# yuliangguo/OmniFusion

Measured on AMD Instinct MI355X. Metric: panoramas/sec at 512x1024 ERP, N=18 256^2 patches; equi2pers+pers2equi GB/s vs HBM peak, higher is better.
Workload: dtype f16x3 (fp16 hi/lo pairs, fp32 accumulate: fp32-class); 1 GPU; cfg2/cfg4 shard: 8 panoramas/GPU/step, 512x1024 ERP, fov 80, nrows 4 (18 patches); full single-pass spherical_fusion forward (confidence=True) at patch size 128 — the only size the reference network exists at (SURVEY 0.1); random-init weights (seed 42); inputs resident in HBM; resample pair at 18x256^2 reported in roofline_resample; per_gpu_batch=8, global_batch=8, parallelism=image-sharded x1, execution=3 forwards in flight per GPU on 3 streams (spherical_fusion.pipelined)

## Files before the change

### omnifusion_amd/csrc/omni_conv_sh.hip

```cpp
#include "omni_conv_sh_common.h"

namespace {

__constant__ float wino_coef[16][4] = {
    {1, 0, 0, 0}, {1, 1, 0, 0}, {1, -1, 0, 0}, {0, -1, 0, 0},
    {1, 0, 1, 0}, {1, 1, 1, 1}, {1, -1, 1, -1}, {0, -1, 0, -1},
    {1, 0, -1, 0}, {1, 1, -1, -1}, {1, -1, -1, 1}, {0, -1, 0, 1},
    {0, 0, -1, 0}, {0, 0, -1, -1}, {0, 0, -1, 1}, {0, 0, 0, 1}};
template <int BM, int BN, int WM, int WN, int NST = 3, int NL = 0, bool PP = false, bool WINO = false, bool X1 = false>
__global__ __launch_bounds__(64 * (WM * WN + NL)) void conv_sh_kernel(ShConvArgs a)
{
    static_assert(!(WINO && X1), "Winograd: f16x3 only");
    static_assert(!PP || (NL > 0 && WM * WN == 8 && NST >= 3), "ping-pong: eight matrix waves (two per SIMD) + loader waves, three stages");
    static_assert(!WINO || (PP && BM / WM == 32 && BN / WN == 32), "Winograd: the ping-pong kernel with 32 x 32 wave tiles");
    constexpr int NW = WM * WN, LW = NL > 0 ? NL : NW, RPP = 8 * LW;
    constexpr int TM = BM / WM / 32, TN = BN / WN / 32;
    constexpr int APASS = BM / RPP, BPASS = BN / RPP, LPS = APASS + BPASS;
    static_assert(APASS >= 1 && BPASS >= 1, "a tile side must cover at least one DMA pass");
    constexpr int A_BYTES = BM * 128, STAGE = (BM + BN) * 128;
    __shared__ __attribute__((aligned(1024))) unsigned char lds[NST * STAGE];
    __shared__ long long cst[OMNI_ABL(32768) ? 256 : 1];
    const bool stamped = OMNI_ABL(32768) && blockIdx.x == 0 && blockIdx.y == 0 && a.ws != nullptr && a.splitk <= 1;
    auto cstamp = [&](int k) { if (OMNI_ABL(32768) && stamped && (threadIdx.x & 63) == 0 && k < 256) cst[k] = clock64(); };
    auto cdump = [&]() { if (OMNI_ABL(32768) && stamped && threadIdx.x == 0) for (int i = 0; i < 256; ++i) reinterpret_cast<long long*>(a.ws)[i] = cst[i]; };
// ... 453 lines not shown
#pragma unroll
    for (int d = 32; d > 0; d >>= 1) q += __shfl_xor(q, d);
    const float rstd = 1.0f / sqrtf(q * (1.0f / 512.0f) + eps);
    const f4v g0 = *reinterpret_cast<const f4v*>(g + lane * 4), g1 = *reinterpret_cast<const f4v*>(g + 256 + lane * 4);
    const f4v b0 = *reinterpret_cast<const f4v*>(b + lane * 4), b1 = *reinterpret_cast<const f4v*>(b + 256 + lane * 4);
    act_store4<SH>(y, o + lane * 4, v0 * rstd * g0 + b0);
    act_store4<SH>(y, o + 256 + lane * 4, v1 * rstd * g1 + b1);
}

__global__ __launch_bounds__(256) void sh_from_f32_kernel(const float* __restrict__ src, void* __restrict__ dst, size_t n4)
{
    const size_t i = (size_t)blockIdx.x * 256 + threadIdx.x;
    if (i >= n4) return;
    h4v hi, lo; sh_split4(*reinterpret_cast<const f4v*>(src + i * 4), hi, lo);
    unsigned char* dp = (unsigned char*)dst + sh_off(i * 4);
    *reinterpret_cast<h4v*>(dp) = hi; *reinterpret_cast<h4v*>(dp + 64) = lo;
}
__global__ __launch_bounds__(256) void sh_to_f32_kernel(const void* __restrict__ src, float* __restrict__ dst, size_t n4)
{
    const size_t i = (size_t)blockIdx.x * 256 + threadIdx.x;
    if (i >= n4) return;
    const unsigned char* sp = (const unsigned char*)src + sh_off(i * 4);
    *reinterpret_cast<f4v*>(dst + i * 4) = sh_join4(*reinterpret_cast<const h4v*>(sp), *reinterpret_cast<const h4v*>(sp + 64));
}

template <bool X1, int BM, int BN, int WM, int WN, int NST = 3, int NL = 0>
void launch_sh(ShConvArgs a, hipStream_t s)
{
    const int tiles = ((a.rows + BM - 1) / BM) * (a.Cout / BN);
    if constexpr (NL > 0 && WM * WN == 8) {
        if (omni_options().conv_pingpong) {
            hipLaunchKernelGGL((conv_sh_kernel<BM, BN, WM, WN, NST, NL, true, false, X1>), dim3(tiles, a.splitk > 1 ? a.splitk : 1), dim3(64 * (WM * WN + NL)), 0, s, a);
            return;
        }
    }
    hipLaunchKernelGGL((conv_sh_kernel<BM, BN, WM, WN, NST, NL, false, false, X1>), dim3(tiles, a.splitk > 1 ? a.splitk : 1), dim3(64 * (WM * WN + NL)), 0, s, a);
}

}

static int conv2d_sh_impl(const void* src1, const void* src2, const void* wt16, const float* bias,
                          const void* res, void* dst, int fmt, int M, int H, int W, int C1, int C2, int Cout,
                          int KH, int KW, int stride, int pad, int act, int splitk, float* ws, size_t ws_bytes,
                          const float* post, size_t post_elems, omni_stream_t stream, bool reduce = true);
extern "C" int omni_conv2d_sh_f16x3_ws(const void* src1, const void* src2, const void* wt16, const float* bias,
                                       const void* res, void* dst, int fmt, int M, int H, int W, int C1, int C2, int Cout,
                                       int KH, int KW, int stride, int pad, int act, int splitk, float* ws, size_t ws_bytes,
                                       omni_stream_t stream)
{
    return conv2d_sh_impl(src1, src2, wt16, bias, res, dst, fmt, M, H, W, C1, C2, Cout, KH, KW, stride, pad, act, splitk, ws, ws_bytes,
                          nullptr, 0, stream);
}
extern "C" int omni_conv2d_sh_f16x3_post_ws(const void* src1, const void* src2, const void* wt16, const float* bias,
                                            const void* res, void* dst, int fmt, int M, int H, int W, int C1, int C2, int Cout,
                                            int KH, int KW, int stride, int pad, int act, int splitk, float* ws, size_t ws_bytes,
                                            const float* post, size_t post_elems, omni_stream_t stream)
{
    return conv2d_sh_impl(src1, src2, wt16, bias, res, dst, fmt, M, H, W, C1, C2, Cout, KH, KW, stride, pad, act, splitk, ws, ws_bytes,
                          post, post_elems, stream);
}
extern "C" int omni_gemm_sh_f16x3_ln512_ws(const void* x, const void* wt16, const float* bias, const float* res, float* tok, const float* ln_g, const float* ln_b,
                                           float eps, void* y, int fmt, int rows, int K, int splitk, float* ws, size_t ws_bytes, omni_stream_t stream)
{
    if (!x || !wt16 || !tok || !ln_g || !ln_b || !y) OMNI_FAIL(OMNI_ERR_INVALID, "omni_gemm_sh_f16x3_ln512: null pointer");
    if (rows <= 0 || K <= 0 || K % 32) OMNI_FAIL(OMNI_ERR_INVALID, "omni_gemm_sh_f16x3_ln512: bad shape");
    if (fmt & 8) OMNI_FAIL(OMNI_ERR_UNSUPPORTED, "omni_gemm_sh_f16x3_ln512: no f16x1 form (fmt bit 3)");
    const int S = std::min(splitk, K / 32);
    if (S < 2) OMNI_FAIL(OMNI_ERR_INVALID, "omni_gemm_sh_f16x3_ln512: needs a split-K plan (splitk >= 2); an unsplit GEMM writes its result in its own epilogue");
    const int rc = conv2d_sh_impl(x, nullptr, wt16, bias, res, tok, 2, rows, 1, 1, K, 0, 512, 1, 1, 1, 0, OMNI_ACT_NONE, S, ws, ws_bytes, nullptr, 0, stream, false);
    if (rc != OMNI_OK) return rc;
    hipStream_t s = (hipStream_t)stream;
    if (fmt & 1) hipLaunchKernelGGL(sh_splitk_reduce_ln512_kernel<true>, dim3((rows + 3) / 4), dim3(256), 0, s, (const float*)ws, bias, res, tok, ln_g, ln_b, y, rows, S, (size_t)rows * 512, eps);
    else         hipLaunchKernelGGL(sh_splitk_reduce_ln512_kernel<false>, dim3((rows + 3) / 4), dim3(256), 0, s, (const float*)ws, bias, res, tok, ln_g, ln_b, y, rows, S, (size_t)rows * 512, eps);
    OMNI_HIP(hipGetLastError());
    return OMNI_OK;
}

template <bool X1>
static void conv_sh_select(const ShConvArgs& a, int fmt, hipStream_t s)
{
    const int KH = a.KH, KW = a.KW, stride = a.stride, pad = a.pad, H = a.H, W = a.W, M = a.M, Cout = a.Cout;
    const int ksteps = KH * KW * ((a.C1 + a.C2) / 32);
    const long long rows = a.rows;
    if (a.splitk <= 1 && KH == 3 && KW == 3 && stride == 1 && pad == 1 && H == W && (W == 16 || (W == 8 && omni_options().conv_img >= 2)) && rows % 128 == 0 &&
        Cout % 64 == 0 && !(fmt & 4) && omni_options().conv_img > 0 && !omni_options().conv_nohalo) {
        const int grid = (int)(rows / 128) * (Cout / 64);
        if (omni_options().conv_halo_bn == 32) {
            if (W == 16) omni_halo_launch(&a, 32, 4, false, 16, X1, 2 * grid, s);
            else         omni_halo_launch(&a, 32, 4, false, 8, X1, 2 * grid, s);
        }
        else if (W == 16) omni_halo_launch(&a, 64, 4, false, 16, X1, grid, s);
        else         omni_halo_launch(&a, 64, 4, false, 8, X1, grid, s);
        return;
    }
    if (a.splitk <= 1 && KH == 3 && KW == 3 && stride == 1 && pad == 1 && W % HT_W == 0 && H % 4 == 0 && !omni_options().conv_nohalo) {
        const int th = (H % 8 == 0 && omni_options().conv_halo_th == 8) ? 8 : 4;
        const int grid = M * (H / th) * (W / HT_W);
        if (th == 8) {
            if (Cout % 64 == 0 && omni_options().conv_halo_bn != 32) omni_halo_launch(&a, 64, 8, false, 0, X1, grid * (Cout / 64), s);
            else                omni_halo_launch(&a, 32, 8, false, 0, X1, grid * (Cout / 32), s);
        } else {
            const bool bn32 = omni_options().conv_halo_bn == 32 || ((fmt & 4) && omni_options().conv_halo_bn_lat == 32);
            if (Cout % 64 == 0 && !bn32) omni_halo_launch(&a, 64, 4, false, 0, X1, grid * (Cout / 64), s);
            else                omni_halo_launch(&a, 32, 4, false, 0, X1, grid * (Cout / 32), s);
        }
        return;
    }
    int tile = omni_options().conv_sh_tile;
    if (tile < 0) tile = 8;
    if (Cout % 64 != 0) launch_sh<X1, 128, 32, 4, 1>(a, s);
    else if (tile == 2 && Cout % 128 == 0) launch_sh<X1, 128, 128, 2, 2>(a, s);
    else if (tile == 1) launch_sh<X1, 128, 64, 2, 2>(a, s);
    else if (tile == 3) launch_sh<X1, 128, 64, 4, 2>(a, s);
    else if (tile == 4 && Cout % 128 == 0) launch_sh<X1, 128, 128, 4, 2>(a, s);
    else if (tile == 8 && Cout % 128 == 0 && ((rows + 255) / 256) * (long long)(Cout / 128) * a.splitk >= std::max(1, omni_options().conv_big_blocks)) launch_sh<X1, 256, 128, 4, 2>(a, s);
    else if (tile == 8 && Cout % 128 == 0 && ((rows + 127) / 128) * (long long)(Cout / 128) * a.splitk >= 128) launch_sh<X1, 128, 128, 4, 2, 3, 4>(a, s);
    else if (tile == 8 && ((rows + 127) / 128) * (long long)(Cout / 64) * a.splitk >= 128) launch_sh<X1, 128, 64, 4, 2, 3, 4>(a, s);
    else if (tile == 9 && Cout % 128 == 0 && ((rows + 255) / 256) * (long long)(Cout / 128) * a.splitk >= 128) launch_sh<X1, 256, 128, 4, 2>(a, s);
    else if (tile == 9 && Cout % 128 == 0 && ((rows + 127) / 128) * (long long)(Cout / 128) * a.splitk >= 128) launch_sh<X1, 128, 128, 4, 2>(a, s);
    else if (tile == 9 && ((rows + 127) / 128) * (long long)(Cout / 64) * a.splitk >= 128) launch_sh<X1, 128, 64, 4, 2>(a, s);
    else if (tile >= 5 && tile <= 7 && Cout % 128 == 0 && ((rows + 127) / 128) * (long long)(Cout / 128) * a.splitk >= (32ll << (tile - 4))) launch_sh<X1, 128, 128, 4, 2>(a, s);
    else if (tile >= 5 && tile <= 7 && ((rows + 127) / 128) * (long long)(Cout / 64) * a.splitk >= (32ll << (tile - 4))) launch_sh<X1, 128, 64, 4, 2>(a, s);
    else if (((rows + 63) / 64) * (long long)(Cout / 64) * a.splitk <= 256 && ksteps >= 8 && !omni_options().conv_nodeep) {
        if (omni_options().conv_deep_loaders) launch_sh<X1, 64, 64, 2, 2, 6, 4>(a, s);
        else launch_sh<X1, 64, 64, 2, 2, 6>(a, s);
    }
    else launch_sh<X1, 64, 64, 2, 2>(a, s);
}

static int conv2d_sh_impl(const void* src1, const void* src2, const void* wt16, const float* bias,
                          const void* res, void* dst, int fmt, int M, int H, int W, int C1, int C2, int Cout,
                          int KH, int KW, int stride, int pad, int act, int splitk, float* ws, size_t ws_bytes,
                          const float* post, size_t post_elems, omni_stream_t stream, bool reduce)
{
    const int dst_sh = fmt & 1;
    if (!src1 || !wt16 || !dst) OMNI_FAIL(OMNI_ERR_INVALID, "omni_conv2d_sh: null pointer");
    if (C1 <= 0 || C1 % 32 || C2 < 0 || C2 % 32 || Cout <= 0 || Cout % 32 || (C2 > 0 && !src2))
        OMNI_FAIL(OMNI_ERR_INVALID, "omni_conv2d_sh: channels must be multiples of 32");
    if (M <= 0 || H <= 0 || W <= 0 || KH <= 0 || KW <= 0 || KH > 3 || KW > 3 || stride <= 0 || pad < 0)
        OMNI_FAIL(OMNI_ERR_INVALID, "omni_conv2d_sh: bad shape (kernels up to 3x3)");
    ShConvArgs a;
    a.src1 = src1; a.src2 = src2; a.wt = wt16; a.bias = bias; a.res = res; a.dst = dst; a.dst_sh = dst_sh; a.res_f32 = (fmt >> 1) & 1;
    a.dbg = 0; a.noxcd = omni_options().conv_noxcd; a.wt_major = 0; a.epi_lds = omni_options().conv_epi_lds && !(fmt & 4);
#ifdef OMNI_DEBUG_BUILD
    a.dbg = omni_debug_bits("OMNI_CONV_DBG");
#endif
    a.M = M; a.H = H; a.W = W; a.C1 = C1; a.C2 = C2; a.Cout = Cout;
    a.KH = KH; a.KW = KW; a.stride = stride; a.pad = pad; a.act = act;
    a.Ho = (H + 2 * pad - KH) / stride + 1; a.Wo = (W + 2 * pad - KW) / stride + 1;
    const long long rows = (long long)M * a.Ho * a.Wo;
    if (rows <= 0 || rows >= (1ll << 31) || (long long)M * H * W >= (1ll << 31))
        OMNI_FAIL(OMNI_ERR_UNSUPPORTED, "omni_conv2d_sh: too many pixels for 32-bit row indices");
    a.rows = (int)rows;
    const int ksteps = KH * KW * ((C1 + C2) / 32);
    if ((long long)M * H * W * (C1 > C2 ? C1 : C2) * 4 >= (1ll << 31) || (long long)Cout * ksteps * 128 >= (1ll << 31))
        OMNI_FAIL(OMNI_ERR_UNSUPPORTED, "omni_conv2d_sh: an operand of 2 GiB or more (32-bit buffer offsets)");
    int S = splitk;
    if (S > ksteps) S = ksteps;
    if (S > 1 && (!ws || ws_bytes < (size_t)S * rows * Cout * sizeof(float)))
        OMNI_FAIL(OMNI_ERR_INVALID, "omni_conv2d_sh: split-K workspace too small");
    a.splitk = S > 1 ? S : 1; a.ws = ws;
    a.wt_major = omni_options().conv_wt_major == 2 || (omni_options().conv_wt_major == 1 &&
                 (long long)Cout * ksteps * 128 > (long long)M * H * W * (C1 + C2) * 4) ? 1 : 0;
    a.post = post; a.post_rows = 1; a.wino_th = a.wino_tw = a.wino_pix = 0;
    if (post) {
        if (Cout <= 0 || post_elems == 0 || post_elems % (size_t)Cout || post_elems / (size_t)Cout > 0x7fffffffull)
            OMNI_FAIL(OMNI_ERR_INVALID, "omni_conv2d_sh: the post-activation addend must hold whole rows of Cout channels");
        if (a.splitk > 1) OMNI_FAIL(OMNI_ERR_UNSUPPORTED, "omni_conv2d_sh: no post-activation addend with split-K");
        a.post_rows = (unsigned)(post_elems / (size_t)Cout);
    }
    hipStream_t s = (hipStream_t)stream;
    if (fmt & 8) conv_sh_select<true>(a, fmt, s);
    else         conv_sh_select<false>(a, fmt, s);
    OMNI_HIP(hipGetLastError());
    if (a.splitk > 1 && reduce) {
        const size_t n4 = (size_t)rows * Cout / 4;
        hipLaunchKernelGGL(sh_splitk_reduce_kernel, dim3((unsigned)((n4 + 255) / 256)), dim3(256), 0, s, (const float*)ws, bias, res, dst,
                           n4, Cout, a.splitk, (size_t)rows * Cout, act, a.dst_sh, a.res_f32);
        OMNI_HIP(hipGetLastError());
    }
    return OMNI_OK;
}

extern "C" int omni_splitk_reduce_ln512(const float* parts, int nparts, const float* bias, const float* res, float* tok, const float* lg, const float* lb,
                                        float eps, void* y, int fmt, int rows, omni_stream_t stream)
{
    if (!parts || nparts < 1 || !tok || !lg || !lb || !y || rows <= 0) OMNI_FAIL(OMNI_ERR_INVALID, "omni_splitk_reduce_ln512: null pointer or empty input");
    hipStream_t s = (hipStream_t)stream;
    if (fmt & 1) hipLaunchKernelGGL(sh_splitk_reduce_ln512_kernel<true>, dim3((rows + 3) / 4), dim3(256), 0, s, parts, bias, res, tok, lg, lb, y, rows, nparts, (size_t)rows * 512, eps);
    else         hipLaunchKernelGGL(sh_splitk_reduce_ln512_kernel<false>, dim3((rows + 3) / 4), dim3(256), 0, s, parts, bias, res, tok, lg, lb, y, rows, nparts, (size_t)rows * 512, eps);
    OMNI_HIP(hipGetLastError());
    return OMNI_OK;
}

OMNI_SH_OVERFLOW_ACCESSOR(omni_sh_overflow_conv)

extern "C" int omni_sh_overflow(int* flag, int reset)
{
    if (!flag) OMNI_FAIL(OMNI_ERR_INVALID, "omni_sh_overflow: null output");
    OMNI_HIP(hipDeviceSynchronize());
    unsigned v = 0;
    if (omni_sh_overflow_conv(&v, reset) != 0 || omni_sh_overflow_halo(&v, reset) != 0 || omni_sh_overflow_up2(&v, reset) != 0 ||
        omni_sh_overflow_rows(&v, reset) != 0 || omni_sh_overflow_net(&v, reset) != 0)
        OMNI_FAIL(OMNI_ERR_HIP, "omni_sh_overflow: could not read the device flag");
    *flag = v ? 1 : 0;
    return OMNI_OK;
}

extern "C" int omni_sh_from_f32(const float* src, void* dst, size_t n, omni_stream_t stream)
{
    if (!src || !dst || n % 32) OMNI_FAIL(OMNI_ERR_INVALID, "omni_sh_from_f32: null pointer or n % 32 != 0");
    if (n == 0) return OMNI_OK;
    hipLaunchKernelGGL(sh_from_f32_kernel, dim3((unsigned)((n / 4 + 255) / 256)), dim3(256), 0, (hipStream_t)stream, src, dst, n / 4);
    OMNI_HIP(hipGetLastError());
    return OMNI_OK;
}
extern "C" int omni_sh_to_f32(const void* src, float* dst, size_t n, omni_stream_t stream)
{
    if (!src || !dst || n % 32) OMNI_FAIL(OMNI_ERR_INVALID, "omni_sh_to_f32: null pointer or n % 32 != 0");
    if (n == 0) return OMNI_OK;
    hipLaunchKernelGGL(sh_to_f32_kernel, dim3((unsigned)((n / 4 + 255) / 256)), dim3(256), 0, (hipStream_t)stream, src, dst, n / 4);
    OMNI_HIP(hipGetLastError());
    return OMNI_OK;
}

namespace {

__global__ __launch_bounds__(256) void wino_input_sh_kernel(const void* __restrict__ src, void* __restrict__ V, int M, int H, int W, int C, size_t nt)
{
    const size_t i = (size_t)blockIdx.x * 256 + threadIdx.x;
    const int cq = C >> 2;
    if (i >= nt * cq) return;
    const size_t tl = i / cq;
    const int c = (int)(i - tl * cq) * 4;
    const int tw = W >> 1, th = H >> 1;
    const int m = (int)(tl / (size_t)(th * tw)), rem = (int)(tl - (size_t)m * th * tw), ty = rem / tw, tx = rem - ty * tw;
    f4v d[4][4];
#pragma unroll
    for (int a_ = 0; a_ < 4; ++a_)
#pragma unroll
        for (int b_ = 0; b_ < 4; ++b_) {
            const int y = 2 * ty - 1 + a_, x = 2 * tx - 1 + b_;
            d[a_][b_] = ((unsigned)y < (unsigned)H && (unsigned)x < (unsigned)W) ? act_load4<true>(src, (((size_t)m * H + y) * W + x) * C + c) : (f4v)(0.0f);
        }
    f4v u[4][4];
#pragma unroll
    for (int b_ = 0; b_ < 4; ++b_) { u[0][b_] = d[0][b_] - d[2][b_]; u[1][b_] = d[1][b_] + d[2][b_]; u[2][b_] = d[2][b_] - d[1][b_]; u[3][b_] = d[1][b_] - d[3][b_]; }
#pragma unroll
    for (int xi = 0; xi < 4; ++xi) {
        const f4v v0 = u[xi][0] - u[xi][2], v1 = u[xi][1] + u[xi][2], v2 = u[xi][2] - u[xi][1], v3 = u[xi][1] - u[xi][3];
        act_store4<true>(V, ((size_t)(4 * xi + 0) * nt + tl) * C + c, v0);
        act_store4<true>(V, ((size_t)(4 * xi + 1) * nt + tl) * C + c, v1);
        act_store4<true>(V, ((size_t)(4 * xi + 2) * nt + tl) * C + c, v2);
        act_store4<true>(V, ((size_t)(4 * xi + 3) * nt + tl) * C + c, v3);
    }
}

}

extern "C" int omni_wino_input_sh(const void* src, void* V, int M, int H, int W, int C, omni_stream_t stream)
{
    if (!src || !V) OMNI_FAIL(OMNI_ERR_INVALID, "omni_wino_input_sh: null pointer");
    if (M <= 0 || H <= 0 || W <= 0 || (H & 1) || (W & 1) || C <= 0 || C % 32) OMNI_FAIL(OMNI_ERR_INVALID, "omni_wino_input_sh: even image sides, channels a multiple of 32");
    const size_t nt = (size_t)M * (H / 2) * (W / 2), n = nt * (C / 4);
    if (16 * nt * C * 4 >= (1ull << 31)) OMNI_FAIL(OMNI_ERR_UNSUPPORTED, "omni_wino_input_sh: the transformed tensor must stay under 2 GiB (32-bit buffer offsets)");
    hipLaunchKernelGGL(wino_input_sh_kernel, dim3((unsigned)((n + 255) / 256)), dim3(256), 0, (hipStream_t)stream, src, V, M, H, W, C, nt);
    OMNI_HIP(hipGetLastError());
    return OMNI_OK;
}

extern "C" int omni_conv3x3_wino_sh_f16x3(const void* V, const void* wt16, const float* bias, const void* res, void* dst, int fmt,
                                          int M, int H, int W, int C, int Cout, int act, int splitk, float* ws, size_t ws_bytes, omni_stream_t stream)
{
    if (!V || !wt16 || !dst) OMNI_FAIL(OMNI_ERR_INVALID, "omni_conv3x3_wino_sh: null pointer");
    if (M <= 0 || H <= 0 || W <= 0 || (H & 1) || (W & 1) || C <= 0 || C % 32 || Cout <= 0 || Cout % 64) OMNI_FAIL(OMNI_ERR_INVALID, "omni_conv3x3_wino_sh: even image sides, C % 32 == 0, Cout % 64 == 0");
    if (splitk != 1 && splitk != 2 && splitk != 4) OMNI_FAIL(OMNI_ERR_INVALID, "omni_conv3x3_wino_sh: splitk must be 1, 2 or 4 (it divides the sixteen positions)");
    if (fmt & 8) OMNI_FAIL(OMNI_ERR_UNSUPPORTED, "omni_conv3x3_wino_sh: no f16x1 form (fmt bit 3)");
    const long long nt = (long long)M * (H / 2) * (W / 2), pix = (long long)M * H * W;
    if (16 * nt * C * 4 >= (1ll << 31) || (long long)Cout * 16 * C * 4 >= (1ll << 31) || pix >= (1ll << 31)) OMNI_FAIL(OMNI_ERR_UNSUPPORTED, "omni_conv3x3_wino_sh: an operand of 2 GiB or more");
    if (splitk > 1 && (!ws || ws_bytes < (size_t)splitk * pix * Cout * sizeof(float))) OMNI_FAIL(OMNI_ERR_INVALID, "omni_conv3x3_wino_sh: split workspace too small");
    ShConvArgs a;
    a.src1 = V; a.src2 = nullptr; a.wt = wt16; a.bias = bias; a.res = res; a.dst = dst; a.dst_sh = fmt & 1; a.res_f32 = (fmt >> 1) & 1;
    a.dbg = 0; a.noxcd = omni_options().conv_noxcd; a.wt_major = 0; a.epi_lds = 0;
    a.M = 1; a.H = 16; a.W = (int)nt; a.C1 = C; a.C2 = 0; a.Cout = Cout; a.KH = 16; a.KW = 1; a.stride = 1; a.pad = 0; a.act = act;
    a.Ho = H; a.Wo = W; a.rows = (int)nt; a.splitk = splitk; a.ws = ws; a.post = nullptr; a.post_rows = 1;
// ... 14 lines not shown
```

### omnifusion_amd/csrc/omni_conv_sh_common.h

```cpp
#pragma once
#include <stdlib.h>
#include <algorithm>
#include <type_traits>
#include "omni_internal.h"
#include "omni_sh.h"

#ifndef OMNI_CONV_ABL
#define OMNI_CONV_ABL 0
#endif
#define OMNI_ABL(bit) ((OMNI_CONV_ABL & (bit)) != 0)
#ifndef OMNI_PP_PRIO
#define OMNI_PP_PRIO 0
#endif
#ifndef OMNI_G1_PW
#define OMNI_G1_PW 4
#endif

namespace {

typedef float f16v __attribute__((ext_vector_type(16)));
typedef float f4v __attribute__((ext_vector_type(4)));
typedef _Float16 h8v __attribute__((ext_vector_type(8)));
typedef _Float16 h4v __attribute__((ext_vector_type(4)));
typedef _Float16 h2v __attribute__((ext_vector_type(2)));
// ... 117 lines not shown
                *reinterpret_cast<f4v*>(tile + px * PITCH + 32 * j + 8 * q + 4 * (lane >> 5)) = v;
            }
    }
    asm volatile("s_waitcnt lgkmcnt(0)" ::: "memory");
    constexpr int TASKS = 32 * NT * 4 / 64;
    constexpr int HALF = TASKS >= 4 ? TASKS / 2 : TASKS;
    const bool post = POST && a.post != nullptr;
#pragma unroll
    for (int k0 = 0; k0 < TASKS; k0 += HALF) {
        f4v va[HALF], vb[HALF], pa[HALF], pb[HALF]; h8v rh[HALF], rl[HALF];
        size_t off[HALF]; bool ok[HALF];
#pragma unroll
        for (int kk = 0; kk < HALF; ++kk) {
            const int task = (k0 + kk) * 64 + lane, px = task / (4 * NT), rem = task - px * (4 * NT), j = rem >> 2, pc = rem & 3;
            ok[kk] = px < nrows;
            va[kk] = *reinterpret_cast<const f4v*>(tile + px * PITCH + 32 * j + 8 * pc);
            vb[kk] = *reinterpret_cast<const f4v*>(tile + px * PITCH + 32 * j + 8 * pc + 4);
            off[kk] = ((px < 16 ? r0 + px : r1 + (px - 16)) * a.Cout + c0[j]) * 4 + 16 * pc;
            if (a.bias) { va[kk] += *reinterpret_cast<const f4v*>(a.bias + c0[j] + 8 * pc); vb[kk] += *reinterpret_cast<const f4v*>(a.bias + c0[j] + 8 * pc + 4); }
            if (a.res && ok[kk]) {
                rh[kk] = *reinterpret_cast<const h8v*>((const unsigned char*)a.res + off[kk]);
                rl[kk] = *reinterpret_cast<const h8v*>((const unsigned char*)a.res + off[kk] + 64);
            }
            if (post && ok[kk]) {
                const float* pp = a.post + (size_t)((unsigned)(px < 16 ? r0 + px : r1 + (px - 16)) % a.post_rows) * a.Cout + c0[j] + 8 * pc;
                pa[kk] = *reinterpret_cast<const f4v*>(pp); pb[kk] = *reinterpret_cast<const f4v*>(pp + 4);
            }
        }
#pragma unroll
        for (int kk = 0; kk < HALF; ++kk) {
            if (!ok[kk]) continue;
            f4v v0 = va[kk], v1 = vb[kk];
            if (a.res) {
#pragma unroll
                for (int e = 0; e < 4; ++e) { v0[e] += fmaf((float)rl[kk][e], 4.8828125e-4f, (float)rh[kk][e]); v1[e] += fmaf((float)rl[kk][4 + e], 4.8828125e-4f, (float)rh[kk][4 + e]); }
            }
            if (a.act == OMNI_ACT_RELU) {
#pragma unroll
                for (int e = 0; e < 4; ++e) { v0[e] = fmaxf(v0[e], 0.f); v1[e] = fmaxf(v1[e], 0.f); }
            } else if (a.act == OMNI_ACT_GELU) {
#pragma unroll
                for (int e = 0; e < 4; ++e) { v0[e] = 0.5f * v0[e] * (1.0f + erff(v0[e] * 0.70710678118654752440f)); v1[e] = 0.5f * v1[e] * (1.0f + erff(v1[e] * 0.70710678118654752440f)); }
            }
            if (post) { v0 += pa[kk]; v1 += pb[kk]; }
            h4v h0, l0, h1, l1;
            sh_split4(v0, h0, l0); sh_split4(v1, h1, l1);
            h8v oh, ol;
#pragma unroll
            for (int e = 0; e < 4; ++e) { oh[e] = h0[e]; oh[4 + e] = h1[e]; ol[e] = l0[e]; ol[4 + e] = l1[e]; }
            *reinterpret_cast<h8v*>((unsigned char*)a.dst + off[kk]) = oh;
            *reinterpret_cast<h8v*>((unsigned char*)a.dst + off[kk] + 64) = ol;
        }
    }
}

__device__ __forceinline__ void splitk_finish(f4v v, size_t o, const float* __restrict__ bias, const void* __restrict__ res, void* __restrict__ dst,
                                              int Cout, int act, int dst_sh, int res_f32)
{
    if (bias) v += *reinterpret_cast<const f4v*>(bias + (o % Cout));
    if (res && res_f32) v += *reinterpret_cast<const f4v*>((const float*)res + o);
    else if (res) {
        const unsigned char* rp = (const unsigned char*)res + sh_off(o);
        v += sh_join4(*reinterpret_cast<const h4v*>(rp), *reinterpret_cast<const h4v*>(rp + 64));
    }
    if (act == OMNI_ACT_RELU) { v.x = fmaxf(v.x, 0.f); v.y = fmaxf(v.y, 0.f); v.z = fmaxf(v.z, 0.f); v.w = fmaxf(v.w, 0.f); }
    else if (act == OMNI_ACT_GELU) {
#pragma unroll
        for (int e = 0; e < 4; ++e) v[e] = 0.5f * v[e] * (1.0f + erff(v[e] * 0.70710678118654752440f));
    }
    if (dst_sh) {
        h4v hi, lo; sh_split4(v, hi, lo);
        unsigned char* dp = (unsigned char*)dst + sh_off(o);
        *reinterpret_cast<h4v*>(dp) = hi; *reinterpret_cast<h4v*>(dp + 64) = lo;
    } else {
        *reinterpret_cast<f4v*>((float*)dst + o) = v;
    }
}

constexpr int HT_W = 32, HPW = HT_W + 2;

}

void omni_halo_launch(const void* args, int bn, int th, bool up2, int iw, bool x1, unsigned grid, hipStream_t s);
int omni_sh_overflow_halo(unsigned* out, int reset);
int omni_sh_overflow_up2(unsigned* out, int reset);
int omni_sh_overflow_rows(unsigned* out, int reset);
int omni_sh_overflow_net(unsigned* out, int reset);
```

### omnifusion_amd/csrc/omni_geometry.hip

```cpp
#include <math.h>
#include <stdlib.h>
#include <string.h>
#include <mutex>
#include <vector>
#include <memory>

#include "omni_internal.h"

static thread_local std::string g_err;
void omni_set_error(const std::string& msg) { g_err = msg; }
extern "C" const char* omni_last_error(void) { return g_err.c_str(); }
extern "C" int omni_version(void) { return OMNI_VERSION; }

namespace {
struct OptName { const char* name; const char* env; int OmniOptions::* field; int dflt; };
const OptName kOpts[] = {
    {"conv_sh_tile", "OMNI_CONV_SH_TILE", &OmniOptions::conv_sh_tile, -1},
    {"conv_nohalo", "OMNI_CONV_NOHALO", &OmniOptions::conv_nohalo, 0},
    {"conv_halo_th", "OMNI_CONV_HALO_TH", &OmniOptions::conv_halo_th, 4},
    {"conv_big_blocks", "OMNI_CONV_BIG_BLOCKS", &OmniOptions::conv_big_blocks, 128},
    {"conv_halo_bn_lat", "OMNI_CONV_HALO_BN_LAT", &OmniOptions::conv_halo_bn_lat, 32},
    {"conv_deep_loaders", "OMNI_CONV_DEEP_LOADERS", &OmniOptions::conv_deep_loaders, 1},
    {"conv_halo_up2_bn_lat", "OMNI_CONV_HALO_UP2_BN_LAT", &OmniOptions::conv_halo_up2_bn_lat, 64},
    {"conv_halo_bn", "OMNI_CONV_HALO_BN", &OmniOptions::conv_halo_bn, 64},
    {"conv_img", "OMNI_CONV_IMG", &OmniOptions::conv_img, 1},
    {"conv_nodeep", "OMNI_CONV_NODEEP", &OmniOptions::conv_nodeep, 0},
    {"conv_pingpong", "OMNI_CONV_PINGPONG", &OmniOptions::conv_pingpong, 1},
    {"conv_noxcd", "OMNI_CONV_NOXCD", &OmniOptions::conv_noxcd, 0},
    {"conv_wt_major", "OMNI_CONV_WT_MAJOR", &OmniOptions::conv_wt_major, 1},
    {"conv_stem_pc", "OMNI_CONV_STEM_PC", &OmniOptions::conv_stem_pc, 1},
    {"conv_epi_lds", "OMNI_CONV_EPI_LDS", &OmniOptions::conv_epi_lds, 1},
    {"conv_up2_persist", "OMNI_CONV_UP2_PERSIST", &OmniOptions::conv_up2_persist, 1},
    {"splitk_max", "OMNI_SPLITK_MAX", &OmniOptions::splitk_max, 0},
    {"e2p_gather", "OMNI_E2P_GATHER", &OmniOptions::e2p_gather, 0},
    {"e2p_notab", "OMNI_E2P_NOTAB", &OmniOptions::e2p_notab, 0},
    {"e2p_verbose", "OMNI_E2P_VERBOSE", &OmniOptions::e2p_verbose, 0},
    {"e2p_bwd_simple", "OMNI_E2P_BWD_SIMPLE", &OmniOptions::e2p_bwd_simple, 0},
    {"p2e_bwd_simple", "OMNI_P2E_BWD_SIMPLE", &OmniOptions::p2e_bwd_simple, 0},
    {"bwd_table_mb", "OMNI_BWD_TABLE_MB", &OmniOptions::bwd_table_mb, 1024},
    {"bwd_wide", "OMNI_BWD_WIDE", &OmniOptions::bwd_wide, 1},
    {"bwd_lmax", "OMNI_BWD_LMAX", &OmniOptions::bwd_lmax, 0},
    {"bwd_chunk", "OMNI_BWD_CHUNK", &OmniOptions::bwd_chunk, 0},
    {"p2e_gather", "OMNI_P2E_GATHER", &OmniOptions::p2e_gather, 0},
    {"e2p_nbuf", "OMNI_E2P_NBUF", &OmniOptions::e2p_nbuf, 0},
    {"e2p_slot_kb", "OMNI_E2P_SLOT_KB", &OmniOptions::e2p_slot_kb, 6},
    {"e2p_tile_h", "OMNI_E2P_TILE_H", &OmniOptions::e2p_tile_h, 0},
    {"e2p_ref_lds", "OMNI_E2P_REF_LDS", &OmniOptions::e2p_ref_lds, 1},
    {"e2p_store", "OMNI_E2P_STORE", &OmniOptions::e2p_store, 1},
    {"e2p_slots", "OMNI_E2P_SLOTS", &OmniOptions::e2p_slots, 0},
    {"e2p_split", "OMNI_E2P_SPLIT", &OmniOptions::e2p_split, 0},
    {"e2p_full", "OMNI_E2P_FULL", &OmniOptions::e2p_full, -1},
    {"e2p_fb_planes", "OMNI_E2P_FB_PLANES", &OmniOptions::e2p_fb_planes, 0},
    {"e2p_fb_pos", "OMNI_E2P_FB_POS", &OmniOptions::e2p_fb_pos, 0},
    {"e2p_region", "OMNI_E2P_REGION", &OmniOptions::e2p_region, 0},
    {"p2e_band", "OMNI_P2E_BAND", &OmniOptions::p2e_band, 0},
    {"p2e_nbuf", "OMNI_P2E_NBUF", &OmniOptions::p2e_nbuf, 0},
    {"p2e_lds_kb", "OMNI_P2E_LDS_KB", &OmniOptions::p2e_lds_kb, 0},
    {"p2e_planes", "OMNI_P2E_PLANES", &OmniOptions::p2e_planes, 0},
    {"p2e_walk", "OMNI_P2E_WALK", &OmniOptions::p2e_walk, 1},
    {"p2e_tile8", "OMNI_P2E_TILE8", &OmniOptions::p2e_tile8, 1},
    {"p2e_store", "OMNI_P2E_STORE", &OmniOptions::p2e_store, 1},
    {"fv_bwd_lds", "OMNI_FV_BWD_LDS", &OmniOptions::fv_bwd_lds, 1},
    {"geom_cache_max", "OMNI_GEOM_CACHE_MAX", &OmniOptions::geom_cache_max, 16},
    {"chamfer_split", "OMNI_CHAMFER_SPLIT", &OmniOptions::chamfer_split, 1},
    {"augment_lut", "OMNI_AUGMENT_LUT", &OmniOptions::augment_lut, 1},
    {"conv_wgrad_rows", "OMNI_CONV_WGRAD_ROWS", &OmniOptions::conv_wgrad_rows, 0},
};
}

OmniOptions& omni_options()
{
    static OmniOptions o = [] {
        OmniOptions v;
        for (const OptName& k : kOpts) {
            const char* e = getenv(k.env);
            v.*(k.field) = e ? (*e ? atoi(e) : 1) : k.dflt;
        }
        return v;
    }();
    return o;
}

int omni_num_cus()
{
    static int cus[64] = {0};
    int dev = 0;
    if (hipGetDevice(&dev) != hipSuccess || dev < 0 || dev >= 64) return 256;
    if (cus[dev] == 0) {
        int n = 0;
        cus[dev] = (hipDeviceGetAttribute(&n, hipDeviceAttributeMultiprocessorCount, dev) == hipSuccess && n > 0) ? n : 256;
    }
    return cus[dev];
}

extern "C" int omni_set_option(const char* name, int value)
{
    if (!name) OMNI_FAIL(OMNI_ERR_INVALID, "omni_set_option: null name");
    for (const OptName& k : kOpts)
        if (strcmp(k.name, name) == 0) { omni_options().*(k.field) = value; return OMNI_OK; }
    OMNI_FAIL(OMNI_ERR_INVALID, std::string("omni_set_option: unknown option '") + name + "'");
}

extern "C" int omni_get_option(const char* name, int* value)
{
    if (!name || !value) OMNI_FAIL(OMNI_ERR_INVALID, "omni_get_option: null argument");
    for (const OptName& k : kOpts)
        if (strcmp(k.name, name) == 0) { *value = omni_options().*(k.field); return OMNI_OK; }
// ... 227 lines not shown
```

### omnifusion_amd/csrc/omni_internal.h

```cpp
#pragma once
#include <mutex>
#include <hip/hip_runtime.h>
#include <hip/hip_fp16.h>
#include <stdint.h>
#include <string>
#include <vector>

#include "../../include/omnifusion.h"

#define OMNI_MAX_PATCH 46
#define OMNI_WAVE 64

void omni_set_error(const std::string& msg);
#define OMNI_FAIL(code, msg) do { omni_set_error(msg); return (code); } while (0)
#define OMNI_HIP(expr) do { hipError_t e_ = (expr); if (e_ != hipSuccess) {                   \
        omni_set_error(std::string(#expr) + ": " + hipGetErrorString(e_)); return OMNI_ERR_HIP; } } while (0)

struct OmniOptions {
    int conv_sh_tile;
    int conv_nohalo;
    int conv_halo_th;
    int conv_halo_bn_lat;
    int conv_halo_up2_bn_lat;
    int conv_deep_loaders;
    int conv_big_blocks;
    int conv_halo_bn;
    int conv_img;
    int conv_nodeep;
    int conv_pingpong;
    int conv_noxcd;
    int conv_wt_major;
    int conv_stem_pc;
    int conv_epi_lds;
    int conv_up2_persist;
    int splitk_max;
    int e2p_gather;
    int e2p_notab;
    int e2p_verbose;
    int e2p_bwd_simple;
    int p2e_bwd_simple;
    int p2e_gather;
    int e2p_nbuf;
    int e2p_store;
    int e2p_slots;
    int e2p_split;
    int e2p_full;
    int e2p_fb_planes;
    int e2p_region;
    int e2p_fb_pos;
    int e2p_ref_lds;
    int e2p_tile_h;
    int e2p_slot_kb;
    int p2e_band;
    int p2e_lds_kb;
    int p2e_nbuf;
    int p2e_planes;
    int p2e_store;
    int p2e_tile8;
    int p2e_walk;
    int bwd_wide;
    int bwd_chunk;
    int bwd_lmax;
    int bwd_table_mb;
    int fv_bwd_lds;
    int geom_cache_max;
    int chamfer_split;
    int augment_lut;
    int conv_wgrad_rows;
};
OmniOptions& omni_options();
int omni_num_cus();

#ifdef OMNI_DEBUG_BUILD
#define OMNI_DBG(a, bit) (((a).dbg & (bit)) != 0)
int omni_debug_bits(const char* env_name);
long long* omni_debug_trace_buf();
#else
#define OMNI_DBG(a, bit) false
#endif

struct PatchTab {
    int   N;
    float lam0[OMNI_MAX_PATCH];
    float slam[OMNI_MAX_PATCH];
    float clam[OMNI_MAX_PATCH];
    float sphi[OMNI_MAX_PATCH];
    float cphi[OMNI_MAX_PATCH];
};

constexpr int OMNI_SP_LMAX = 48;
struct OmniSpTable {
    uint2* ent = nullptr; int* slice_off = nullptr; int* cnt = nullptr;
    uint2* long_ent = nullptr; int* long_off = nullptr; int* long_row = nullptr;
    int nrows = 0, nslices = 0, nlong = 0, ok = 0;
    long long nent = 0, npadded = 0, nlong_ent = 0;
};
void omni_sp_free(OmniSpTable& t);
struct omni_geometry;
int omni_bwd_workspace(omni_geometry* g, hipStream_t stream, size_t bytes, float** out);

struct omni_geometry {
    int device;
    int pinned;
    int nrows, N;
    float fov_h, fov_w;
    int ph, pw, H, W;
    PatchTab e2p;
    PatchTab p2e;
    float center_p[2 * OMNI_MAX_PATCH];
// ... 71 lines not shown
```

### omnifusion_amd/isa.py

```python
import os
import re
import subprocess
import sys
import tempfile

LLVM = os.environ.get("OMNI_LLVM_BIN", "/opt/rocm/lib/llvm/bin")
TARGET = "hipv4-amdgcn-amd-amdhsa--gfx950"
FORBIDDEN = re.compile(r"\bv_pk_(mul|add|fma)_f32\b")
COUNTED = ("e2p_box_kernel", "p2e_lds_kernel", "p2e_walk_kernel", "e2p_ref_kernel")
HOT = ("conv_sh_kernel", "conv3x3_halo_sh_kernel", "conv3x3_up2_g1_kernel", "stem_f16x3_pc_kernel", "heads_kernel", "maxpool_kernel",
       "layernorm512_kernel", "attention_kernel", "upsample_sh8_kernel")
HOST_ONLY = ("omni_png.o", "omni_geometry.o")


def _device_object(obj, tmp):
    fat = os.path.join(tmp, "fat.bin")
    co = os.path.join(tmp, "dev.co")
    r = subprocess.run([os.path.join(LLVM, "llvm-objcopy"), "--dump-section", f".hip_fatbin={fat}", obj, os.path.join(tmp, "copy.o")],
                       stderr=subprocess.DEVNULL)
    if r.returncode != 0 or not os.path.exists(fat) or os.path.getsize(fat) == 0:
        return None
    subprocess.check_call([os.path.join(LLVM, "clang-offload-bundler"), "--unbundle", "--type=o", f"--input={fat}",
                           f"--targets={TARGET}", f"--output={co}"])
    return co


def disassemble(obj):
    with tempfile.TemporaryDirectory() as tmp:
        co = _device_object(obj, tmp)
        if co is None:
            return ""
        return subprocess.check_output([os.path.join(LLVM, "llvm-objdump"), "-d", "--mcpu=gfx950", co]).decode()


def kernel_meta(obj):
    with tempfile.TemporaryDirectory() as tmp:
        co = _device_object(obj, tmp)
        if co is None:
            return []
        txt = subprocess.check_output([os.path.join(LLVM, "llvm-readelf"), "--notes", co]).decode()
    out, cur = [], None
    keys = {".vgpr_count": "vgpr", ".agpr_count": "agpr", ".sgpr_count": "sgpr", ".group_segment_fixed_size": "lds",
            ".private_segment_fixed_size": "scratch", ".vgpr_spill_count": "vgpr_spill", ".sgpr_spill_count": "sgpr_spill",
            ".name": "name"}
    for line in txt.splitlines():
        m = re.match(r"^  - \.(\w+):\s*(\S+)\s*$", line)
        if m:
            cur = {}
            out.append(cur)
            line = "    ." + m.group(1) + ": " + m.group(2)
        m = re.match(r"^    (\.\w+):\s*(\S+)\s*$", line)
        if m and cur is not None and m.group(1) in keys:
            v = m.group(2)
            cur[keys[m.group(1)]] = v if m.group(1) == ".name" else int(v)
    return [k for k in out if "name" in k]


def demangle(names):
    try:
        p = subprocess.run([os.path.join(LLVM, "llvm-cxxfilt")], input="\n".join(names).encode(), stdout=subprocess.PIPE, check=True)
        return p.stdout.decode().splitlines()
    except Exception:
        return list(names)


def objects():
    from . import build as b
    return [s[:-4] + ".o" for s in b.sources()]


def check(objs=None):
    bad = []
    found = {c: 0 for c in COUNTED + HOT}
    full = objs is None
    for obj in objs or objects():
        base = os.path.basename(obj)
        if not os.path.exists(obj):
            bad.append(f"{base}: object missing (build first)")
            continue
        asm = disassemble(obj)
        if not asm.strip():
            if base not in HOST_ONLY:
                bad.append(f"{base}: no gfx950 device code could be extracted (not in HOST_ONLY): the ISA rules were NOT checked")
            continue
        cur = "?"
        for line in asm.splitlines():
            if line.endswith(">:"):
                cur = line.split("<", 1)[1][:-2]
            elif FORBIDDEN.search(line):
                bad.append(f"{base}: packed-fp32 instruction in {cur}: {line.strip()[:80]}")
                break
        for k in kernel_meta(obj):
            for c in COUNTED + HOT:
# ... 39 lines not shown
```

Before: 4103 panoramas/s.

## Add 3x3 halo conv kernel with 64-pixel wave tiles and 4-deep weight ring

Adds a new 3x3 halo convolution kernel in which each of four waves computes two 32-pixel row tiles across 64 output channels (8-row tiles, or whole 16x16 images). The full input halo is staged once per channel group and weights stream through a four-buffer LDS ring three stages ahead. It is enabled by default (conv_halo_w64=1) for wide maps and takes priority over the existing halo paths. This is meant to raise reuse of each weight tile across more pixels and keep two blocks resident per CU. The cost is extra register pressure, a hand-counted wait schedule, and a barrier-heavy reload at every channel-group boundary.

New measurement: 4127 panoramas/s, median of 6. Within noise of the previous version (+0.6%).

```diff
diff --git a/omnifusion_amd/csrc/omni_conv_halo_w64.hip b/omnifusion_amd/csrc/omni_conv_halo_w64.hip
--- /dev/null
+++ b/omnifusion_amd/csrc/omni_conv_halo_w64.hip
@@ -0,0 +1,189 @@
+#include <stdio.h>
+#include <string.h>
+#include "omni_conv_sh_common.h"
+
+namespace {
+
+template <int BN, int IW, bool ROWS>
+__global__ __launch_bounds__(256, 2) void conv3x3_halo_w64_sh_kernel(ShConvArgs a)
+{
+    static_assert(BN == 64 && (IW == 0 || IW == 16), "64 output channels per block; wide maps or 16 x 16 images");
+    constexpr int TN = BN / 32, NP = 2, NW = 4, RPP = 8 * NW, TH = 8;
+    constexpr int HROW = IW > 0 ? IW + 2 : HPW;
+    constexpr int HPX = IW > 0 ? (IW + 2) * (IW + 2) : (TH + 2) * HPW, HA_INSTR = (HPX * 8 + 63) / 64, HA_BYTES = HA_INSTR * 1024;
+    constexpr int APASS = (HA_INSTR + NW - 1) / NW;
+    constexpr int NB = 4, AHEAD = NB - 1, B_BYTES = BN * 128, BPASS = BN / RPP;
+    static_assert(BN % RPP == 0, "every wave issues the same number of weight pieces per stage: the waits below count them");
+    static_assert(HA_BYTES + NB * B_BYTES <= 80 * 1024, "two blocks per CU");
+    __shared__ __attribute__((aligned(1024))) unsigned char lds[HA_BYTES + NB * B_BYTES];
+
+    const int t = threadIdx.x, lane = t & 63, wave = t >> 6;
+    const int ntn = a.Cout / BN, tw = IW > 0 ? 1 : a.W / HT_W, th = IW > 0 ? 1 : a.H / TH;
+    int bid = a.noxcd ? blockIdx.x : omni_xcd_remap(blockIdx.x, gridDim.x);
+    const int tile_n = bid % ntn; bid /= ntn;
+    const int tx = bid % tw; bid /= tw;
+    const int ty = bid % th; const int m = bid / th;
+    const int y0 = ty * TH, x0 = tx * HT_W, col0 = tile_n * BN;
+    const int G1 = a.C1 >> 5, G = (a.C1 + a.C2) >> 5, ksteps = 9 * G;
+
+    const int gs = (lane & 15) ^ ((4 * wave + (lane >> 4)) & 15);
+    const int rl = 8 * wave + 2 * (lane >> 4) + (gs >> 3), pc16 = (gs & 7) * 16;
+    int wbase[BPASS];
+#pragma unroll
+    for (int i = 0; i < BPASS; ++i) wbase[i] = (col0 + rl + RPP * i) * ksteps * 128 + pc16;
+    const rsrc_t rs1 = make_rsrc(a.src1, (size_t)a.M * a.H * a.W * a.C1 * 4);
+    const rsrc_t rs2 = make_rsrc(a.src2 ? a.src2 : a.src1, a.src2 ? (size_t)a.M * a.H * a.W * a.C2 * 4 : 0);
+    const rsrc_t rsw = make_rsrc(a.wt, (size_t)a.Cout * ksteps * 128);
+
+    auto issue_a = [&](int g) {
+        const bool first = g < G1;
+        const int cs4 = (first ? a.C1 : a.C2) * 4;
+        const int soff = (first ? g : g - G1) * 128 + pc16;
+        unsigned char* sb = lds + wave * 1024;
+        int rz = rl;
+        asm volatile("" : "+v"(rz));
+#pragma unroll
+        for (int i = 0; i < APASS; ++i) {
+            if (wave + NW * i < HA_INSTR) {
+                const int p = rz + RPP * i, hy = p / HROW, hx = p - hy * HROW;
+                int pix;
+                bool in;
+                if constexpr (IW > 0) {
+                    const int iy = hy - 1, ix = hx - 1;
+                    in = p < HPX && (unsigned)iy < (unsigned)IW && (unsigned)ix < (unsigned)IW; pix = (m * IW + iy) * IW + ix;
+                } else {
+                    const int iy = y0 - 1 + hy, ix = x0 - 1 + hx;
+                    in = p < HPX && (unsigned)iy < (unsigned)a.H && (unsigned)ix < (unsigned)a.W; pix = (m * a.H + iy) * a.W + ix;
+                }
+                const int off = in ? pix * cs4 + soff : (int)0x80000000;
+                if (first) dma16(rs1, sb + i * (1024 * NW), off, 0);
+                else       dma16(rs2, sb + i * (1024 * NW), off, 0);
+            }
+        }
+    };
+    auto issue_b = [&](int g, int tap, int buf) {
+        unsigned char* sb = lds + HA_BYTES + buf * B_BYTES + wave * 1024;
+        const int soff = (tap * G + g) * 128;
+#pragma unroll
+        for (int i = 0; i < BPASS; ++i) dma16(rsw, sb + i * (1024 * NW), wbase[i], soff);
+    };
+
+    int pb[NP];
+#pragma unroll
+    for (int q = 0; q < NP; ++q) {
+        if constexpr (IW > 0) {
+            const int tp = 64 * wave + 32 * q + (lane & 31), y = tp / IW, x = tp - y * IW;
+            pb[q] = y * HROW + x;
+        } else pb[q] = (2 * wave + q) * HROW + (lane & 31);
+    }
+    auto pix_off = [&](int p) { const int d = p >> 1; return d * 256 + ((((p & 1) * 8 + (lane >> 5)) ^ (d & 15)) * 16); };
+    int fo[4];
+    {
+        const int r = lane & 31, v = r >> 1, h = lane >> 5;
+#pragma unroll
+        for (int k = 0; k < 4; ++k) fo[k] = v * 256 + ((((r & 1) * 8 + 2 * k + h) ^ v) * 16);
+    }
+
+    f16v acc[NP][TN], acc1[NP][TN];
+#pragma unroll
+    for (int q = 0; q < NP; ++q)
+#pragma unroll
+        for (int j = 0; j < TN; ++j) { acc[q][j] = (f16v)(0.0f); acc1[q][j] = (f16v)(0.0f); }
+
+    issue_a(0);
+#pragma unroll
+    for (int s = 0; s < AHEAD; ++s) issue_b(0, s, s);
+    for (int g = 0; g < G; ++g) {
+#pragma unroll
+        for (int tap = 0; tap < 9; ++tap) {
+            int a0[NP];
+#pragma unroll
+            for (int q = 0; q < NP; ++q) {
+                int p = pb[q];
+                asm volatile("" : "+v"(p));
+                a0[q] = pix_off(p + (tap / 3) * HROW + tap % 3);
+            }
+            if (g + 1 < G || tap + AHEAD <= 9) wait_vm<(AHEAD - 1) * BPASS>();
+            else if (tap == 7)                 wait_vm<BPASS>();
+            else                               wait_vm<0>();
+            static_assert(AHEAD == 3, "the tail above is written for three stages ahead");
+            wait_lds_reads();
+            __builtin_amdgcn_s_barrier();
+            asm volatile("" ::: "memory");
+            const bool more = tap + AHEAD < 9 || g + 1 < G;
+            if (tap == 0 && g > 0) {
+                issue_a(g);
+                issue_b(g, AHEAD, (g * 9 + AHEAD) & (NB - 1));
+                wait_vm<BPASS>();
+                __builtin_amdgcn_s_barrier();
+                asm volatile("" ::: "memory");
+            } else if (more) {
+                if (tap + AHEAD < 9) issue_b(g, tap + AHEAD, (g * 9 + tap + AHEAD) & (NB - 1));
+                else                 issue_b(g + 1, tap + AHEAD - 9, (g * 9 + tap + AHEAD) & (NB - 1));
+            }
+            const unsigned char* sB = lds + HA_BYTES + ((g * 9 + tap) & (NB - 1)) * B_BYTES;
+            h8v bh[2][TN], bl[2][TN], ah[2][NP], al[2][NP];
+#pragma unroll
+            for (int kc = 0; kc < 2; ++kc) {
+#pragma unroll
+                for (int j = 0; j < TN; ++j) {
+                    bh[kc][j] = *reinterpret_cast<const h8v*>(sB + j * (32 * 128) + fo[kc]);
+                    bl[kc][j] = *reinterpret_cast<const h8v*>(sB + j * (32 * 128) + fo[2 + kc]);
+                }
+#pragma unroll
+                for (int q = 0; q < NP; ++q) {
+                    ah[kc][q] = *reinterpret_cast<const h8v*>(lds + (a0[q] ^ (kc * 32)));
+                    al[kc][q] = *reinterpret_cast<const h8v*>(lds + (a0[q] ^ (64 + kc * 32)));
+                }
+            }
+            __builtin_amdgcn_sched_barrier(0);
+#pragma unroll
+            for (int kc = 0; kc < 2; ++kc)
+#pragma unroll
+                for (int q = 0; q < NP; ++q)
+#pragma unroll
+                    for (int j = 0; j < TN; ++j) {
+                        acc[q][j] = __builtin_amdgcn_mfma_f32_32x32x16_f16(bh[kc][j], ah[kc][q], acc[q][j], 0, 0, 0);
+                        acc1[q][j] = __builtin_amdgcn_mfma_f32_32x32x16_f16(bl[kc][j], ah[kc][q], acc1[q][j], 0, 0, 0);
+                        acc1[q][j] = __builtin_amdgcn_mfma_f32_32x32x16_f16(bh[kc][j], al[kc][q], acc1[q][j], 0, 0, 0);
+                    }
+        }
+    }
+
+    int te = threadIdx.x;
+    asm volatile("" : "+v"(te));
+    const int lane_e = te & 63, wave_e = te >> 6;
+    int c0[TN];
+#pragma unroll
+    for (int j = 0; j < TN; ++j) c0[j] = col0 + j * 32;
+    if constexpr (!ROWS) {
+        static_assert(NW * 32 * (32 * TN + 4) * 4 <= (int)sizeof(lds), "the transposition tiles must fit the K loop's buffers");
+        wait_lds_reads();
+        __syncthreads();
+    }
+#pragma unroll
+    for (int q = 0; q < NP; ++q) {
+        const int r0 = IW > 0 ? m * (IW * IW) + 64 * wave_e + 32 * q : (m * a.H + y0 + 2 * wave_e + q) * a.W + x0;
+        if constexpr (!ROWS) {
+            epilogue_tile_lds<TN, true, false>(acc[q], acc1[q], a, (size_t)r0, 32, c0, lane_e, reinterpret_cast<float*>(lds) + wave_e * (32 * (32 * TN + 4)));
+            asm volatile("s_waitcnt lgkmcnt(0)" ::: "memory");
+        } else epilogue_row<TN, 1, false>(acc[q], acc1[q], a, (size_t)(r0 + (lane_e & 31)), c0, lane_e, a.dst_sh != 0);
+    }
+}
+
+}
+
+OMNI_SH_OVERFLOW_ACCESSOR(omni_sh_overflow_halo_w64)
+
+void omni_halo_w64_launch(const void* args, int iw, unsigned grid, hipStream_t s)
+{
+    ShConvArgs a;
+    memcpy(&a, args, sizeof(a));
+    const bool rows = !(a.dst_sh && !a.res_f32 && a.epi_lds);
+#define OMNI_W64(IW, ROWS) \
+    if (iw == IW && rows == ROWS) { hipLaunchKernelGGL((conv3x3_halo_w64_sh_kernel<64, IW, ROWS>), dim3(grid), dim3(256), 0, s, a); return; }
+    OMNI_W64(0, false) OMNI_W64(0, true) OMNI_W64(16, false) OMNI_W64(16, true)
+#undef OMNI_W64
+    fprintf(stderr, "omni_halo_w64_launch: no conv3x3_halo_w64_sh_kernel<64, %d>\n", iw);
+    abort();
+}
diff --git a/omnifusion_amd/csrc/omni_conv_sh.hip b/omnifusion_amd/csrc/omni_conv_sh.hip
--- a/omnifusion_amd/csrc/omni_conv_sh.hip
+++ b/omnifusion_amd/csrc/omni_conv_sh.hip
@@ -559,6 +559,14 @@
     const int KH = a.KH, KW = a.KW, stride = a.stride, pad = a.pad, H = a.H, W = a.W, M = a.M, Cout = a.Cout;
     const int ksteps = KH * KW * ((a.C1 + a.C2) / 32);
     const long long rows = a.rows;
+    if constexpr (!X1) {
+        const int w64 = omni_options().conv_halo_w64;
+        if (w64 && a.splitk <= 1 && KH == 3 && KW == 3 && stride == 1 && pad == 1 && Cout % 64 == 0 && !(fmt & 4) && !omni_options().conv_nohalo &&
+            omni_options().conv_halo_bn != 32) {
+            if ((w64 & 2) && H == 16 && W == 16 && omni_options().conv_img > 0) { omni_halo_w64_launch(&a, 16, (unsigned)(M * (Cout / 64)), s); return; }
+            if ((w64 & 1) && W % HT_W == 0 && H % 8 == 0) { omni_halo_w64_launch(&a, 0, (unsigned)(M * (H / 8) * (W / HT_W) * (Cout / 64)), s); return; }
+        }
+    }
     if (a.splitk <= 1 && KH == 3 && KW == 3 && stride == 1 && pad == 1 && H == W && (W == 16 || (W == 8 && omni_options().conv_img >= 2)) && rows % 128 == 0 &&
         Cout % 64 == 0 && !(fmt & 4) && omni_options().conv_img > 0 && !omni_options().conv_nohalo) {
         const int grid = (int)(rows / 128) * (Cout / 64);
@@ -677,7 +685,7 @@
     if (!flag) OMNI_FAIL(OMNI_ERR_INVALID, "omni_sh_overflow: null output");
     OMNI_HIP(hipDeviceSynchronize());
     unsigned v = 0;
-    if (omni_sh_overflow_conv(&v, reset) != 0 || omni_sh_overflow_halo(&v, reset) != 0 || omni_sh_overflow_up2(&v, reset) != 0 ||
+    if (omni_sh_overflow_conv(&v, reset) != 0 || omni_sh_overflow_halo(&v, reset) != 0 || omni_sh_overflow_halo_w64(&v, reset) != 0 || omni_sh_overflow_up2(&v, reset) != 0 ||
         omni_sh_overflow_rows(&v, reset) != 0 || omni_sh_overflow_net(&v, reset) != 0)
         OMNI_FAIL(OMNI_ERR_HIP, "omni_sh_overflow: could not read the device flag");
     *flag = v ? 1 : 0;
diff --git a/omnifusion_amd/csrc/omni_conv_sh_common.h b/omnifusion_amd/csrc/omni_conv_sh_common.h
--- a/omnifusion_amd/csrc/omni_conv_sh_common.h
+++ b/omnifusion_amd/csrc/omni_conv_sh_common.h
@@ -223,7 +223,9 @@
 }
 
 void omni_halo_launch(const void* args, int bn, int th, bool up2, int iw, bool x1, unsigned grid, hipStream_t s);
+void omni_halo_w64_launch(const void* args, int iw, unsigned grid, hipStream_t s);
 int omni_sh_overflow_halo(unsigned* out, int reset);
+int omni_sh_overflow_halo_w64(unsigned* out, int reset);
 int omni_sh_overflow_up2(unsigned* out, int reset);
 int omni_sh_overflow_rows(unsigned* out, int reset);
 int omni_sh_overflow_net(unsigned* out, int reset);
diff --git a/omnifusion_amd/csrc/omni_geometry.hip b/omnifusion_amd/csrc/omni_geometry.hip
--- a/omnifusion_amd/csrc/omni_geometry.hip
+++ b/omnifusion_amd/csrc/omni_geometry.hip
@@ -23,6 +23,7 @@
     {"conv_deep_loaders", "OMNI_CONV_DEEP_LOADERS", &OmniOptions::conv_deep_loaders, 1},
     {"conv_halo_up2_bn_lat", "OMNI_CONV_HALO_UP2_BN_LAT", &OmniOptions::conv_halo_up2_bn_lat, 64},
     {"conv_halo_bn", "OMNI_CONV_HALO_BN", &OmniOptions::conv_halo_bn, 64},
+    {"conv_halo_w64", "OMNI_CONV_HALO_W64", &OmniOptions::conv_halo_w64, 1},
     {"conv_img", "OMNI_CONV_IMG", &OmniOptions::conv_img, 1},
     {"conv_nodeep", "OMNI_CONV_NODEEP", &OmniOptions::conv_nodeep, 0},
     {"conv_pingpong", "OMNI_CONV_PINGPONG", &OmniOptions::conv_pingpong, 1},
diff --git a/omnifusion_amd/csrc/omni_internal.h b/omnifusion_amd/csrc/omni_internal.h
--- a/omnifusion_amd/csrc/omni_internal.h
+++ b/omnifusion_amd/csrc/omni_internal.h
@@ -25,6 +25,7 @@
     int conv_deep_loaders;
     int conv_big_blocks;
     int conv_halo_bn;
+    int conv_halo_w64;
     int conv_img;
     int conv_nodeep;
     int conv_pingpong;
diff --git a/omnifusion_amd/isa.py b/omnifusion_amd/isa.py
--- a/omnifusion_amd/isa.py
+++ b/omnifusion_amd/isa.py
@@ -8,7 +8,7 @@
 TARGET = "hipv4-amdgcn-amd-amdhsa--gfx950"
 FORBIDDEN = re.compile(r"\bv_pk_(mul|add|fma)_f32\b")
 COUNTED = ("e2p_box_kernel", "p2e_lds_kernel", "p2e_walk_kernel", "e2p_ref_kernel")
-HOT = ("conv_sh_kernel", "conv3x3_halo_sh_kernel", "conv3x3_up2_g1_kernel", "stem_f16x3_pc_kernel", "heads_kernel", "maxpool_kernel",
+HOT = ("conv_sh_kernel", "conv3x3_halo_sh_kernel", "conv3x3_halo_w64_sh_kernel", "conv3x3_up2_g1_kernel", "stem_f16x3_pc_kernel", "heads_kernel", "maxpool_kernel",
        "layernorm512_kernel", "attention_kernel", "upsample_sh8_kernel")
 HOST_ONLY = ("omni_png.o", "omni_geometry.o")
 
```
